# zakuro-ai/asr

Measured on AMD Instinct MI355X. Metric: utterances/sec (10 s, 161-bin) DS2 5x1024 BiGRU CTC train step, higher is better.
Workload: dtype bf16

## Files before the change

### asr_amd/_lib.py

```python
from __future__ import annotations

import ctypes as C
import os
from typing import Optional

_HERE = os.path.dirname(os.path.abspath(__file__))
LIB_PATH = os.environ.get("DS2_LIB_PATH") or os.path.join(_HERE, "lib", "libds2hip.so")

_lib: Optional[C.CDLL] = None

vp, i32, i64, f32, f64, sz = C.c_void_p, C.c_int, C.c_longlong, C.c_float, C.c_double, C.c_size_t

SIGNATURES = {
    "ds2_version": (C.c_char_p, []),
    "ds2_last_error": (C.c_char_p, []),
    "ds2_device_info": (i32, [C.POINTER(i32), C.POINTER(i32), C.c_char_p, i32]),
    "ds2_debug_flags": (i32, [vp, i32]),
    "ds2_rnn_ctx_init": (i32, [vp, vp, vp, vp]),
    "ds2_memset_async": (i32, [vp, i32, sz, vp]),
    "ds2_ablation_build": (i32, []),
    "ds2_rnn_persistent_status": (i32, [vp, vp]),
    "ds2_rnn_persistent_counters": (i32, [vp, vp]),
    "ds2_rnn_poison_if_starved": (i32, [vp, vp, sz, vp]),
    "ds2_rnn_poison_seen": (i32, [vp]),
# ... 32 lines not shown
    "ds2_bn1d_apply_f32": (i32, [vp, i32, vp, i32, i32, i32, vp, vp, vp, vp, f32, vp]),
    "ds2_bn1d_apply_bf16": (i32, [vp, i32, vp, i32, i32, i32, vp, vp, vp, vp, f32, vp]),
    "ds2_bn1d_bwd_f32": (i32, [vp, i32, vp, i32, vp, i32, i32, i32, vp, vp, vp, f32, vp, vp, vp, sz, vp]),
    "ds2_bn1d_bwd_xbf16": (i32, [vp, i32, vp, i32, vp, i32, i32, i32, vp, vp, vp, f32, vp, vp, vp, sz, vp]),
    "ds2_center_colstats": (i32, [vp, i32, vp, i32, vp, i32, vp, i32, i32, i32, vp, vp, vp, vp, vp, f32, vp, sz, vp]),
    "ds2_wih_fold_bf16": (i32, [vp, i32, vp, i32, i32, vp, vp, vp, vp, f32, vp, i32, vp, vp, vp, vp]),
    "ds2_scale_rank1_f32": (i32, [vp, i32, i32, i32, vp, vp, vp, vp]),
    "ds2_chanreduce_workspace_bytes": (sz, [i32]),
    "ds2_bn2d_stats_f32": (i32, [vp, i32, i32, i32, i32, vp, vp, vp, vp, f32, vp, sz, vp]),
    "ds2_bn2d_act_fwd_f32": (i32, [vp, vp, i32, i32, i32, i32, vp, vp, vp, vp, vp, f32, vp]),
    "ds2_bn2d_act_bwd_f32": (i32, [vp, vp, vp, i32, i32, i32, i32, vp, vp, vp, vp, vp, f32, vp, vp, vp, sz, vp]),
    "ds2_bn2d_act_fwd_fused": (i32, [vp, i32, i32, i32, vp, vp, vp, vp, vp, f32, vp, vp, vp, vp]),
    "ds2_bn2d_act_collapse": (i32, [vp, i32, i32, i32, vp, vp, vp, vp, vp, f32, vp, vp, i32, vp]),
    "ds2_bn2d_act_bwd_fused_workspace_bytes": (sz, [i32, i32, i32]),
    "ds2_bn2d_act_bwd_fused": (i32, [vp, vp, i32, i32, i32, vp, vp, vp, vp, vp, f32, vp, vp, vp, vp, vp, vp, vp, sz, vp]),
    "ds2_transpose_bft_f32": (i32, [vp, vp, i32, i32, i32, i32, vp]),
    "ds2_transpose2d_f32": (i32, [vp, i32, i64, vp, i32, i64, i32, i32, i32, vp]),
    "ds2_conv_dims": (None, [i32, i32, C.POINTER(i32), C.POINTER(i32), C.POINTER(i32)]),
    "ds2_conv_packed_floats": (sz, [i32]),
    "ds2_conv_pack_f32": (i32, [vp, vp, vp, vp, vp, vp]),
    "ds2_conv1_fwd_f32": (i32, [vp, vp, vp, vp, vp, i32, i32, i32, vp]),
    "ds2_conv2_fwd_f32": (i32, [vp, vp, vp, vp, vp, i32, i32, i32, vp]),
    "ds2_conv2_dgrad_f32": (i32, [vp, vp, vp, i32, i32, i32, vp]),
    "ds2_conv_wgrad_workspace_bytes": (sz, [i32, i32, i32]),
    "ds2_conv1_wgrad_f32": (i32, [vp, vp, vp, vp, i32, i32, i32, i32, vp, sz, vp]),
    "ds2_conv2_wgrad_f32": (i32, [vp, vp, vp, vp, i32, i32, i32, i32, vp, sz, vp]),
    "ds2_conv2_bf16_packed_bytes": (sz, [i32]),
    "ds2_conv2_pack_bf16": (i32, [vp, vp, vp, vp, vp]),
    "ds2_nhwc_bf16_f32": (i32, [vp, vp, i32, i32, i32, vp]),
    "ds2_conv2_fwd_bf16": (i32, [vp, vp, vp, vp, vp, i32, i32, i32, vp]),
# ... 58 lines not shown
    "ds2_ctc_hot_pack": (i32, [i32, i32, vp, vp, vp, vp, vp, vp, i32, vp, sz]),
    "ds2_ctc_hot_step": (i32, [vp, i32, i32, C.POINTER(i32), C.POINTER(f32)]),
    "ds2_ctc_beam_decode_hot_f32": (i32, [vp, i64, i64, i32, i32, i32, vp, i32, i32, i32, f32, vp, sz, i32, i32, i32, f32, f32, vp, vp, sz,
                                          vp, vp, vp, vp, vp, sz, vp]),
    "ds2_edit_distance_workspace_bytes": (sz, [i32, i64]),
    "ds2_edit_distance_i32": (i32, [vp, i64, vp, vp, vp, vp, i32, i64, vp, vp, sz, vp]),
    "ds2_edit_align_workspace_bytes": (sz, [i32, i64]),
    "ds2_edit_align_i32": (i32, [vp, i64, vp, vp, vp, vp, i32, i64, vp, vp, vp, vp, sz, vp]),
    "ds2_conv1_bf16_row_pitch": (i32, [i32]),
    "ds2_conv1_bf16_bytes": (sz, [i32, i32, i32, i32]),
    "ds2_conv1_pack_bf16": (i32, [vp, vp, vp]),
    "ds2_conv1_gather_bf16": (i32, [vp, vp, vp, i32, i32, i32, vp]),
    "ds2_conv1_fwd_bf16": (i32, [vp, vp, vp, vp, vp, i32, i32, i32, vp]),
    "ds2_conv1_wgrad_bf16_workspace_bytes": (sz, [i32, i32]),
    "ds2_conv1_wgrad_bf16": (i32, [vp, vp, vp, vp, i32, i32, i32, vp, sz, vp]),
    "ds2_spectrogram_frames": (i32, [i32, i32]),
    "ds2_spectrogram_workspace_bytes": (sz, [i32, i32, i32, i32]),
    "ds2_spectrogram_f32": (i32, [vp, i64, vp, i32, i32, i32, i32, vp, i32, i32, vp, vp, sz, vp]),
    "ds2_spectrogram_aug_workspace_bytes": (sz, [i32, i32, i32, i32]),
    "ds2_spectrogram_aug_f32": (i32, [vp, i64, vp, i32, i32, i32, i32, vp, i32, i32, vp, i64, vp, vp, vp, vp, vp, i32, vp, i32, vp, vp, sz,
                                      vp]),
    "ds2_tempo_sizes": (i32, [i32, f64, f64, f64, C.POINTER(i32), C.POINTER(i32), C.POINTER(i32)]),
    "ds2_tempo_out_samples": (i32, [i32, f64]),
    "ds2_tempo_workspace_bytes": (sz, [i32]),
    "ds2_tempo_gain_f32": (i32, [vp, i64, vp, vp, vp, i32, i32, f64, f64, f64, vp, i64, vp, vp, i32, vp, sz, vp]),
    "ds2_wave_unpack_f32": (i32, [vp, i64, i32, vp, vp, vp, i32, i32, vp, i64, vp]),
    "ds2_resample_out_samples": (i64, [i64, i32, i32]),
    "ds2_resample_tile_samples": (i32, []),
    "ds2_wave_resample_f32": (i32, [vp, i64, i32, vp, vp, vp, vp, vp, vp, vp, vp, i64, i32, i32, vp, i64, vp]),
    "ds2_reverb_max_taps": (i32, []),
# ... 57 lines not shown
```

### asr_amd/csrc/conv1_bf16.hip

```cpp
#include "common.h"
#include <type_traits>

namespace {

typedef __bf16 bf16x8 __attribute__((ext_vector_type(8)));
typedef unsigned int u32x4 __attribute__((ext_vector_type(4)));
typedef float f32x4_c1 __attribute__((ext_vector_type(4), aligned(4)));

constexpr int KD = 41, KTAPS = 11, PD = 20, PT = 5, CO = 32, NC = 16;

__device__ __attribute__((aligned(16))) float g_zero_c1[4] = {0.f, 0.f, 0.f, 0.f};

#ifdef DS2_C1_TRACE
__device__ unsigned long long g_c1_trace[8192 * 8];
#define C1T_DECL unsigned long long c1t_[8] = {0, 0, 0, 0, 0, 0, 0, 0}, c1t_last_ = __builtin_amdgcn_s_memtime()
#define C1T(k) do { const unsigned long long n_ = __builtin_amdgcn_s_memtime(); c1t_[k] += n_ - c1t_last_; c1t_last_ = n_; } while (0)
#define C1T_DUMP(blk) do { if (threadIdx.x == 0) for (int k_ = 0; k_ < 8; ++k_) g_c1_trace[(long long)(blk) * 8 + k_] = c1t_[k_]; } while (0)
#else
#define C1T_DECL
#define C1T(k)
#define C1T_DUMP(blk)
#endif

__global__ __launch_bounds__(256) void conv1_gather_kernel(const float* __restrict__ x, __bf16* __restrict__ X16, __bf16* __restrict__ X16T,
// ... 196 lines not shown

constexpr int W_TT = 64;
constexpr int W_PF = 4;
constexpr int W_PITCH = W_TT * 2 + 16;
constexpr int W_SLOT = NC * W_PITCH;
constexpr int W_NR = 44;
constexpr int W_DY = CO * W_PITCH;
constexpr int W_LDS = (W_NR + 1) * W_SLOT + 2 * W_DY;
constexpr int W_TILES = (KD + 1) / 2;
constexpr int W_TPW = (W_TILES + 3) / 4;

struct C1WArgs {
  const __bf16* X16T; const float* dy; const int* lens; float* part;
  int B, F, T, Tp, D1;
};

__global__ __launch_bounds__(256) void conv1_bf16_wgrad_kernel(C1WArgs a) {
  extern __shared__ __attribute__((aligned(16))) char lds[];
  char* ring = lds;
  char* zslot = lds + W_NR * W_SLOT;
  char* dyl = zslot + W_SLOT;
  const int tid = threadIdx.x, lane = tid & 63;
  const int wave = __builtin_amdgcn_readfirstlane(tid >> 6);
  const int l31 = lane & 31, half = lane >> 5;
  const int t0 = blockIdx.x * W_TT, b = blockIdx.y;
  const int len = a.lens ? min(a.lens[b], a.T) : a.T;
  float* out = a.part + ((long long)b * gridDim.x + blockIdx.x) * (CO * KD * KTAPS);

  f32x16 acc[W_TPW];
#pragma unroll
  for (int i = 0; i < W_TPW; ++i)
#pragma unroll
// ... 7 lines not shown
    auto dy_load = [&](int o, int k, f32x4& v) {
      const int co = k >> 4, tq = t0 + (k & 15) * 4;
      const bool row_ok = o < a.D1;
      const float* p = a.dy + (((long long)b * CO + co) * a.D1 + (row_ok ? o : 0)) * a.T + tq;
      const float* z = g_zero_c1;
      v.x = *((row_ok && tq < a.T) ? p : z);
      v.y = *((row_ok && tq + 1 < a.T) ? p + 1 : z);
      v.z = *((row_ok && tq + 2 < a.T) ? p + 2 : z);
      v.w = *((row_ok && tq + 3 < a.T) ? p + 3 : z);
    };
    auto dy_store = [&](int buf, int k, const f32x4& v) {
      typedef __bf16 bf16x4 __attribute__((ext_vector_type(4)));
      const int co = k >> 4, tq = (k & 15) * 4;
      *reinterpret_cast<bf16x4*>(dyl + buf * W_DY + co * W_PITCH + tq * 2) = bf16x4{(__bf16)v.x, (__bf16)v.y, (__bf16)v.z, (__bf16)v.w};
    };
    for (int c = tid; c < W_SLOT / 16; c += 256) *reinterpret_cast<u32x4*>(zslot + c * 16) = u32x4{0u, 0u, 0u, 0u};
    for (int c = tid; c < KD * 128; c += 256) {
      const int r = c >> 7, k = c & 127;
      *reinterpret_cast<u32x4*>(ring + r * W_SLOT + (k >> 3) * W_PITCH + (k & 7) * 16) = *reinterpret_cast<const u32x4*>(row_src(r - PD, k >> 3, k & 7));
    }
    {
      f32x4 v0, v1;
      dy_load(0, tid, v0);
      dy_load(0, tid + 256, v1);
      dy_store(0, tid, v0);
      dy_store(0, tid + 256, v1);
    }
    struct Regs { u32x4 nr; f32x4 d0, d1; };
    const int nrow = tid >> 7, nk = tid & 127;
    unsigned dyoff[2][4];
#pragma unroll
    for (int h = 0; h < 2; ++h) {
      const int k = tid + 256 * h, co = k >> 4, tq = t0 + (k & 15) * 4;
#pragma unroll
      for (int j = 0; j < 4; ++j) dyoff[h][j] = (unsigned)(((long long)co * a.D1 * a.T + min(tq + j, a.T - 1)) * 4);
    }
    const unsigned rowoff = (unsigned)((((long long)nrow * NC + (nk >> 3)) * a.Tp + t0 + (nk & 7) * 8) * 2);
    const char* dy_b = reinterpret_cast<const char*>(a.dy + (long long)b * CO * a.D1 * a.T);
    const char* x_b = reinterpret_cast<const char*>(a.X16T + (long long)b * a.F * NC * a.Tp);
    const int nrow_u = __builtin_amdgcn_readfirstlane(nrow);
    const bool full_tile = t0 + W_TT <= a.T;
    auto fetch = [&](int o, Regs& r, auto full_c) {
      const int f = 2 * o - 1 + PD + nrow_u;
      const bool ok = f < a.F;
      const char* xs = ok ? x_b + (long long)f * NC * a.Tp * 2 - (long long)nrow_u * NC * a.Tp * 2 : reinterpret_cast<const char*>(g_zero_c1);
      r.nr = *reinterpret_cast<const u32x4*>(xs + (ok ? rowoff : 0u));
      const char* ds_ = dy_b + (long long)min(o, a.D1 - 1) * a.T * 4;
      if constexpr (decltype(full_c)::value) {
        const f32x4_c1 q0 = *reinterpret_cast<const f32x4_c1*>(ds_ + dyoff[0][0]), q1 = *reinterpret_cast<const f32x4_c1*>(ds_ + dyoff[1][0]);
        r.d0 = f32x4{q0.x, q0.y, q0.z, q0.w};
        r.d1 = f32x4{q1.x, q1.y, q1.z, q1.w};
      } else {
        r.d0 = f32x4{*reinterpret_cast<const float*>(ds_ + dyoff[0][0]), *reinterpret_cast<const float*>(ds_ + dyoff[0][1]),
                     *reinterpret_cast<const float*>(ds_ + dyoff[0][2]), *reinterpret_cast<const float*>(ds_ + dyoff[0][3])};
        r.d1 = f32x4{*reinterpret_cast<const float*>(ds_ + dyoff[1][0]), *reinterpret_cast<const float*>(ds_ + dyoff[1][1]),
                     *reinterpret_cast<const float*>(ds_ + dyoff[1][2]), *reinterpret_cast<const float*>(ds_ + dyoff[1][3])};
      }
    };
    auto publish = [&](int o, const Regs& r) {
      if (o < a.D1) {
        const int slot = (2 * o - 1 + nrow + 2 * PD) % W_NR;
        *reinterpret_cast<u32x4*>(ring + slot * W_SLOT + (nk >> 3) * W_PITCH + (nk & 7) * 16) = r.nr;
        dy_store(o & 1, tid, r.d0);
        dy_store(o & 1, tid + 256, r.d1);
      }
    };
    auto compute = [&](int o) {
      const char* ap = dyl + (o & 1) * W_DY + l31 * W_PITCH + half * 16;
      const int cl = l31 & 15, kdl = l31 >> 4;
      const int s0 = (2 * o + 2 * wave + kdl) % W_NR;
      const char* bp[W_TPW];
#pragma unroll
      for (int i = 0; i < W_TPW; ++i) {
        const int kd = 2 * (wave + 4 * i) + kdl;
        int slot = s0 + 8 * i;
        slot -= (slot >= W_NR) ? W_NR : 0;
        slot -= (slot >= W_NR) ? W_NR : 0;
        bp[i] = (kd < KD ? ring + slot * W_SLOT : zslot) + cl * W_PITCH + half * 16;
      }
// ... 27 lines not shown
            fetch(o + k + W_PF, rs[k], full_c);
            C1T(1);
            compute(o + k);
            C1T(2);
            publish(o + k + 1, rs[(k + 1) % W_PF]);
            C1T(3);
            __syncthreads();
            C1T(4);
          }
        }
      }
      C1T_DUMP(4096 + (long long)blockIdx.y * gridDim.x + blockIdx.x);
    };
    if (full_tile) run(std::true_type{});
    else run(std::false_type{});
  }
#pragma unroll
  for (int i = 0; i < W_TPW; ++i) {
    const int j = wave + 4 * i;
    if (j < W_TILES) {
      const int kd = 2 * j + (l31 >> 4), c = l31 & 15;
      if (kd < KD && c < KTAPS) {
#pragma unroll
        for (int r = 0; r < 16; ++r) {
          const int co = (r & 3) + 8 * (r >> 2) + 4 * half;
          out[(co * KD + kd) * KTAPS + c] = acc[i][r];
        }
      }
    }
  }
// ... 92 lines not shown

extern "C" size_t ds2_conv1_wgrad_bf16_workspace_bytes(int B, int Tin) {
  const int T = (Tin + 2 * PT - KTAPS) / 2 + 1;
  return (size_t)B * ceil_div(T, W_TT) * CO * KD * KTAPS * sizeof(float);
}

extern "C" int ds2_conv1_wgrad_bf16(const void* X16T, const float* dy1, const int* lens_dev, float* dW1, int B, int F, int Tin, void* ws,
                                    size_t ws_bytes, void* stream) {
  DS2_REQUIRE(X16T && dy1 && dW1 && ws, "ds2_conv1_wgrad_bf16: null pointer");
  DS2_REQUIRE(ws_bytes >= ds2_conv1_wgrad_bf16_workspace_bytes(B, Tin), "ds2_conv1_wgrad_bf16: workspace too small");
  C1WArgs a{};
  a.X16T = (const __bf16*)X16T; a.dy = dy1; a.lens = lens_dev; a.part = (float*)ws;
  a.B = B; a.F = F; a.T = (Tin + 2 * PT - KTAPS) / 2 + 1; a.Tp = pad64(a.T); a.D1 = (F + 2 * PD - KD) / 2 + 1;
  static bool attr_set = false;
  if (!attr_set) {
    DS2_HIP(hipFuncSetAttribute((const void*)conv1_bf16_wgrad_kernel, hipFuncAttributeMaxDynamicSharedMemorySize, W_LDS));
    attr_set = true;
  }
  hipStream_t s = (hipStream_t)stream;
  const int ntt = ceil_div(a.T, W_TT);
  hipLaunchKernelGGL(conv1_bf16_wgrad_kernel, dim3(ntt, B), dim3(256), W_LDS, s, a);
  DS2_LAUNCH_CHECK("conv1_bf16_wgrad_kernel");
  hipLaunchKernelGGL(conv1_wgrad_reduce_kernel, dim3(ceil_div(CO * KD * KTAPS, 32)), dim3(256), 0, s, (const float*)ws, dW1, ntt * B);
  DS2_LAUNCH_CHECK("conv1_wgrad_reduce_kernel");
  return 0;
}
```

### asr_amd/csrc/norm.hip

```cpp
#include "common.h"
#include <algorithm>

namespace {

typedef float f32x4_dw __attribute__((ext_vector_type(4), aligned(4)));
typedef __bf16 nbf16x4 __attribute__((ext_vector_type(4)));
constexpr int BN_ROWS_PER_BLOCK = 32;
__device__ __forceinline__ f32x4 ld4(const float* __restrict__ p, int valid, bool vec) {
  f32x4 v = {0.f, 0.f, 0.f, 0.f};
  if (valid >= 4 && vec) {
    v = *reinterpret_cast<const f32x4*>(p);
  } else if (valid >= 4) {
    const f32x4_dw q = *reinterpret_cast<const f32x4_dw*>(p);
    v.x = q.x; v.y = q.y; v.z = q.z; v.w = q.w;
  } else {
    if (valid > 0) v.x = p[0];
    if (valid > 1) v.y = p[1];
    if (valid > 2) v.z = p[2];
    if (valid > 3) v.w = p[3];
  }
  return v;
}
__device__ __forceinline__ void st4(float* __restrict__ p, f32x4 v, int valid, bool vec) {
  if (valid >= 4 && vec) {
// ... 322 lines not shown
    } else {
#pragma unroll
      for (int j = 0; j < 4; ++j)
        if (tq0 + j < T) {
          y[j] = Yraw[row * T + tq0 + j];
          if (BWD) da[j] = dA[row * T + tq0 + j];
        }
    }
    float r[4];
#pragma unroll
    for (int j = 0; j < 4; ++j) {
      const bool live = tq0 + j < len;
      if (!BWD) {
        r[j] = live ? fminf(fmaxf((y[j] - mu) * (rs * ga) + be, 0.f), 20.f) : 0.f;
      } else {
        const float xh = (y[j] - mu) * rs;
        const float z = xh * ga + be;
        const float dz = (live && z > 0.f && z < 20.f) ? da[j] : 0.f;
        r[j] = live ? ga * rs * (dz - s0[c] * inv_count - xh * (s1[c] * inv_count)) : 0.f;
      }
      tile[c][tl4 + j] = r[j];
    }
    if (out_f32) {
      if (full4) *reinterpret_cast<f32x4u*>(out_f32 + row * T + tq0) = f32x4u{r[0], r[1], r[2], r[3]};
      else {
#pragma unroll
        for (int j = 0; j < 4; ++j) if (tq0 + j < T) out_f32[row * T + tq0 + j] = r[j];
      }
    }
    if (out_pad) {
#pragma unroll
      for (int j = 0; j < 4; ++j) if (tq0 + j < T) out_pad[row * Tp + 8 + tq0 + j] = (nbf16)r[j];
      if (blockIdx.x == 0 && l16 < 8) out_pad[row * Tp + l16] = (nbf16)0.f;
      if (blockIdx.x == gridDim.x - 1) for (int q = l16; T + 8 + q < Tp; q += 16) out_pad[row * Tp + T + 8 + q] = (nbf16)0.f;
// ... 651 lines not shown
                                      const float* var, const float* gamma, const float* beta, float eps, float* dgamma, float* dbeta,
                                      float* dbias, float* dy_f32, void* dy_pad, void* dy_nhwc, void* ws, size_t ws_bytes, void* stream) {
  DS2_REQUIRE(Y && dA && lens_dev && mean && var && gamma && beta && dgamma && dbeta && dbias, "ds2_bn2d_act_bwd_fused: null pointer");
  DS2_REQUIRE(ws && ws_bytes >= ds2_bn2d_act_bwd_fused_workspace_bytes(B, D, T), "ds2_bn2d_act_bwd_fused: workspace too small");
  const size_t red_bytes = ds2_chanreduce_workspace_bytes(32);
  int rc = chan_reduce_launch(1, Y, dA, B, 32, D, T, lens_dev, mean, var, gamma, beta, eps, 1, dbeta, dgamma, nullptr, nullptr, 0.f, ws,
                              red_bytes, (hipStream_t)stream);
  if (rc) return rc;
  float* part = reinterpret_cast<float*>(static_cast<char*>(ws) + red_bytes);
  const int Tp = (T + 16 + 7) / 8 * 8;
  const dim3 grid(ceil_div(T, 64), D, B);
  hipLaunchKernelGGL((bn2d_tile_kernel<true>), grid, dim3(256), 0, (hipStream_t)stream, Y, dA, B, D, T, Tp, lens_dev, mean, var, gamma, beta,
                     (const float*)dbeta, (const float*)dgamma, eps, 1.0f / ((float)B * D * T), dy_f32, (nbf16*)dy_pad, (nbf16*)dy_nhwc, part);
  DS2_LAUNCH_CHECK("bn2d_tile_kernel<bwd>");
  const long long nparts = (long long)grid.x * grid.y * grid.z;
  double* tmp = reinterpret_cast<double*>(reinterpret_cast<char*>(part) + align_up((size_t)nparts * 32 * sizeof(float), 16));
  const long long rpb = (nparts + CPF_BLOCKS - 1) / CPF_BLOCKS;
  const int nblk = (int)((nparts + rpb - 1) / rpb);
  hipLaunchKernelGGL(chan_part_finalize_kernel, dim3(nblk), dim3(256), 0, (hipStream_t)stream, (const float*)part, nparts, rpb, tmp, nblk, dbias, 0);
  hipLaunchKernelGGL(chan_part_finalize_kernel, dim3(1), dim3(256), 0, (hipStream_t)stream, (const float*)part, nparts, rpb, tmp, nblk, dbias, 1);
  DS2_LAUNCH_CHECK("chan_part_finalize_kernel");
  return 0;
}

extern "C" int ds2_transpose_bft_f32(const float* src, float* dst, int B, int F, int T, int dir, void* stream) {
  DS2_REQUIRE(src && dst && B > 0 && F > 0 && T > 0, "ds2_transpose_bft_f32: bad args");
  dim3 grid(ceil_div(T, 64), ceil_div(F, 64), B);
  hipLaunchKernelGGL(transpose_bft_kernel, grid, dim3(256), 0, (hipStream_t)stream, src, dst, B, F, T, dir);
  DS2_LAUNCH_CHECK("transpose_bft_kernel");
  return 0;
}

extern "C" int ds2_transpose2d_f32(const float* src, int ld_src, long long stride_src, float* dst, int ld_dst, long long stride_dst,
                                   int R, int Cc, int batch, void* stream) {
  DS2_REQUIRE(src && dst && R > 0 && Cc > 0 && batch > 0, "ds2_transpose2d_f32: bad args");
  dim3 grid(ceil_div(Cc, 32), ceil_div(R, 32), batch);
  hipLaunchKernelGGL(transpose2d_kernel, grid, dim3(256), 0, (hipStream_t)stream, src, ld_src, stride_src, dst, ld_dst, stride_dst, R, Cc);
// ... 4 lines not shown
```

### asr_amd/engine.py

```python
from __future__ import annotations

from dataclasses import dataclass, field
from typing import Dict, List, Optional

import torch

from . import _lib, ops

Tensor = torch.Tensor
import os as _os
def _tune(name: str, default: str) -> str:
    return _os.environ.get(name, default) if _os.environ.get("DS2_EXPERIMENTAL") == "1" else default


OVERLAP_MODE = _tune("DS2_OVERLAP", "2")
OVERLAP_WGRAD = OVERLAP_MODE == "1"
WGRAD_TN = _tune("DS2_WGRAD_TN", "1") != "0"
CONV_STATS = _tune("DS2_CONV_STATS", "1") != "0"
FUSE_BN_BWD = _tune("DS2_FUSE_BN_BWD", "1") != "0"
WGRAD_SIDE = _tune("DS2_WGRAD_SIDE", "sk")
WGRAD_IDLE = _tune("DS2_WGRAD_IDLE", "1") != "0"
WGRAD_IDLE_MIN_CUS = int(_tune("DS2_WGRAD_IDLE_MIN_CUS", "64"))
F32_GEMM = _os.environ.get("DS2_F32_GEMM", "split")


F32_RNN = _os.environ.get("DS2_F32_RNN", "split")


F32_CONV = _os.environ.get("DS2_F32_CONV", "split")
F32_CONV_FWD = _tune("DS2_F32_CONV_FWD", "f32")
CONV2_WGRAD = _tune("DS2_CONV2_WGRAD", "nhwc")
GX_BF16 = _tune("DS2_GX_BF16", "0") != "0"
WS_PREARM = _tune("DS2_WS_PREARM", "1") != "0"
BN_FOLD = _tune("DS2_BN_FOLD", "1") != "0"
BN_FOLD_IDLE = _tune("DS2_BN_FOLD_IDLE", "1") != "0"


def _f32_split_ok(M: int, N: int, K: int, H: int = 8) -> bool:
    return F32_GEMM == "split" and M >= 512 and N >= 256 and K >= 256 and K % 8 == 0 and N % 8 == 0 and H % 8 == 0


_BWD_PERSISTENT = {}
_SIDE = {}


def _idle_cus_beside_bwd_recurrence(device, B: int, H: int) -> int:
# ... 652 lines not shown
    cp = "conv.seq_module."
    da2 = ops.transpose_bft(dy, B, 32 * D2, T, to_tbf=False).view(B, 32, D2, T)
    m2, v2 = ctx.st2
    bf = cfg.precision == "bf16"
    if bf:
        _, dy2p, dy2n = ops.bn2d_act_bwd_fused(ctx.y2, da2, lens_dev, m2, v2, W[cp + "4.weight"], W[cp + "4.bias"], Gr[cp + "4.weight"],
                                               Gr[cp + "4.bias"], Gr[cp + "3.bias"], want_pad=CONV2_WGRAD != "nhwc", want_nhwc=True)
        del da2
        if CONV2_WGRAD == "nhwc":
            ops.conv2_wgrad_nhwc_bf16(ctx.a1p, dy2n, lens_dev, Gr[cp + "3.weight"])
        else:
            ops.conv2_wgrad_bf16(ctx.a1p, dy2p, lens_dev, Gr[cp + "3.weight"], T)
        da1 = ops.conv2_dgrad_bf16(dy2n, ctx.packs[1], ctx.packs[2], D1)
        del dy2p, dy2n
        m1, v1 = ctx.st1
        dy1, _, _ = ops.bn2d_act_bwd_fused(ctx.y1, da1, lens_dev, m1, v1, W[cp + "1.weight"], W[cp + "1.bias"], Gr[cp + "1.weight"],
                                           Gr[cp + "1.bias"], Gr[cp + "0.bias"], want_f32=True)
        del da1
        ops.conv1_wgrad_bf16(ctx.x16t, dy1, lens_dev, Gr[cp + "0.weight"], ctx.x.shape[3])
        ctx.x16t = None
    elif F32_CONV == "split":
        dy2, dy2p, dy2n = ops.bn2d_act_bwd_fused(ctx.y2, da2, lens_dev, m2, v2, W[cp + "4.weight"], W[cp + "4.bias"], Gr[cp + "4.weight"],
                                                 Gr[cp + "4.bias"], Gr[cp + "3.bias"], want_f32=True, want_pad=True, want_nhwc=True)
        del da2
        r2 = ops.bf16_residual(dy2)
        del dy2
        dy2p_lo, dy2n_lo = ops.padcast_bf16(r2), ops.nhwc_bf16(r2)
        r2 = ops.bf16_residual(ctx.a1)
        a1p = (ops.padcast_bf16(ctx.a1), ops.padcast_bf16(r2))
        del r2
        ph = ops.conv2_pack_bf16(W[cp + "3.weight"])
        pl = ops.conv2_pack_bf16(ops.bf16_residual(W[cp + "3.weight"]))
        g2 = Gr[cp + "3.weight"]
        gb, gc = torch.empty_like(g2), torch.empty_like(g2)
# ... 33 lines not shown
```

### asr_amd/ops.py

```python
from __future__ import annotations

import ctypes as C
import math
import threading
from typing import Optional, Tuple

import numpy as np
import torch

from . import _lib

Tensor = torch.Tensor
BN_EPS = 1e-5
BN_MOMENTUM = 0.1


def _ptr(t: Optional[Tensor]):
    return None if t is None else t.data_ptr()


def _stream():
    return torch.cuda.current_stream().cuda_stream


# ... 605 lines not shown
    _chk_f32(Y, dA, mean, var, gamma, beta, dgamma, dbeta, dbias)
    lib = _lib.load()
    B, Cc, D, T = Y.shape
    assert Cc == 32 and Y.is_contiguous() and dA.is_contiguous() and dA.shape == Y.shape
    d32 = torch.empty_like(Y) if want_f32 else None
    dpad = torch.empty(B, 32, D, lib.ds2_conv_padded_pitch(T), dtype=torch.bfloat16, device=Y.device) if want_pad else None
    dnh = torch.empty(B, D, T, 32, dtype=torch.bfloat16, device=Y.device) if want_nhwc else None
    wsb = lib.ds2_bn2d_act_bwd_fused_workspace_bytes(B, D, T)
    ws = _ws(wsb, Y.device)
    _lib.check(lib.ds2_bn2d_act_bwd_fused(Y.data_ptr(), dA.data_ptr(), B, D, T, lens_dev.data_ptr(), mean.data_ptr(), var.data_ptr(),
                                          gamma.data_ptr(), beta.data_ptr(), BN_EPS, dgamma.data_ptr(), dbeta.data_ptr(), dbias.data_ptr(),
                                          _ptr(d32), _ptr(dpad), _ptr(dnh), ws.data_ptr(), wsb, _stream()), "ds2_bn2d_act_bwd_fused")
    return d32, dpad, dnh


def chan_sum(Y: Tensor) -> Tensor:
    mean, _ = bn2d_stats(Y)
    B, Cc, D, T = Y.shape
    return mean * float(B * D * T)


def transpose_bft(src: Tensor, B: int, F: int, T: int, to_tbf: bool) -> Tensor:
    _chk_f32(src)
    dst = torch.empty((T, B, F) if to_tbf else (B, F, T), dtype=torch.float32, device=src.device)
    _lib.check(_lib.load().ds2_transpose_bft_f32(src.data_ptr(), dst.data_ptr(), B, F, T, 0 if to_tbf else 1, _stream()),
               "ds2_transpose_bft_f32")
    return dst


def transpose_batched(src: Tensor) -> Tensor:
# ... 99 lines not shown


def chanstats_from_partials(part: Tensor, count: int, run_mean: Optional[Tensor] = None, run_var: Optional[Tensor] = None):
    _chk_f32(part, run_mean, run_var)
    nblk, Cc, _ = part.shape
    mean = torch.empty(Cc, dtype=torch.float32, device=part.device)
    var = torch.empty_like(mean)
    lib = _lib.load()
    wsb = lib.ds2_chanstats_from_partials_workspace_bytes()
    ws = _ws(wsb, part.device)
    _lib.check(lib.ds2_chanstats_from_partials(part.data_ptr(), nblk, Cc, float(count), mean.data_ptr(), var.data_ptr(), _ptr(run_mean),
                                               _ptr(run_var), BN_MOMENTUM, ws.data_ptr(), wsb, _stream()), "ds2_chanstats_from_partials")
    return mean, var


def conv1_wgrad_bf16(X16T: Tensor, dy1: Tensor, lens_dev: Tensor, dW1: Tensor, Tin: int):
    _chk_f32(dy1, dW1)
    lib = _lib.load()
    B, F = X16T.shape[0], X16T.shape[1]
    wsb = lib.ds2_conv1_wgrad_bf16_workspace_bytes(B, Tin)
    ws = _ws(wsb, dy1.device)
    _lib.check(lib.ds2_conv1_wgrad_bf16(X16T.data_ptr(), dy1.data_ptr(), lens_dev.data_ptr(), dW1.data_ptr(), B, F, Tin, ws.data_ptr(), wsb,
                                        _stream()), "ds2_conv1_wgrad_bf16")


def conv2_pack_bf16(w2: Tensor):
    _chk_f32(w2)
    lib = _lib.load()
    bufs = [torch.empty(lib.ds2_conv2_bf16_packed_bytes(i), dtype=torch.uint8, device=w2.device) for i in range(3)]
    _lib.check(lib.ds2_conv2_pack_bf16(w2.data_ptr(), bufs[0].data_ptr(), bufs[1].data_ptr(), bufs[2].data_ptr(), _stream()),
               "ds2_conv2_pack_bf16")
    return tuple(bufs)


# ... 1040 lines not shown
```

### include/ds2hip.h

```cpp
#ifndef DS2HIP_H
#define DS2HIP_H

#include <stddef.h>
#include <stdint.h>

#ifdef __cplusplus
extern "C" {
#endif

const char* ds2_version(void);
const char* ds2_last_error(void);
int ds2_device_info(int* cu_count, int* wave_size, char* arch, int arch_len);
int ds2_ablation_build(void);

typedef struct ds2_rnn_ctx {
  int size;
  int persist_fwd, persist_bwd;
  int cooldown;
  int rearm_calls;
  int starved_total;
  int last_path;
  int last_bwd_kind;
  int debug_flags;
  int ws_prearmed;
// ... 66 lines not shown
                       float momentum, void* ws, size_t ws_bytes, void* stream);
int ds2_bn2d_act_fwd_f32(const float* Y, float* A, int B, int C, int D, int T, const int* lens_dev, const float* mean,
                         const float* var, const float* gamma, const float* beta, float eps, void* stream);
int ds2_bn2d_act_bwd_f32(const float* Y, const float* dA, float* dY, int B, int C, int D, int T, const int* lens_dev, const float* mean,
                         const float* var, const float* gamma, const float* beta, float eps, float* dgamma, float* dbeta, void* ws,
                         size_t ws_bytes, void* stream);

int ds2_bn2d_act_fwd_fused(const float* Y, int B, int D, int T, const int* lens_dev, const float* mean, const float* var,
                           const float* gamma, const float* beta, float eps, float* a_f32, void* a_pad, void* a_nhwc, void* stream);
int ds2_bn2d_act_collapse(const float* Y, int B, int D, int T, const int* lens_dev, const float* mean, const float* var,
                          const float* gamma, const float* beta, float eps, float* x_f32, void* x_bf16, int ld_bf, void* stream);
size_t ds2_bn2d_act_bwd_fused_workspace_bytes(int B, int D, int T);
int ds2_bn2d_act_bwd_fused(const float* Y, const float* dA, int B, int D, int T, const int* lens_dev, const float* mean,
                           const float* var, const float* gamma, const float* beta, float eps, float* dgamma, float* dbeta,
                           float* dbias, float* dy_f32, void* dy_pad, void* dy_nhwc, void* ws, size_t ws_bytes, void* stream);
int ds2_transpose_bft_f32(const float* src, float* dst, int B, int F, int T, int dir, void* stream);
int ds2_transpose2d_f32(const float* src, int ld_src, long long stride_src, float* dst, int ld_dst, long long stride_dst, int R, int Cc,
                        int batch, void* stream);

void ds2_conv_dims(int F, int Tin, int* D1, int* D2, int* T);
size_t ds2_conv_packed_floats(int which );
int ds2_conv_pack_f32(const float* w1, const float* w2, float* wpk1, float* wpk2, float* wpk2d, void* stream);
int ds2_conv1_fwd_f32(const float* x, const float* wpk1, const float* bias, const int* lens_dev, float* y1, int B, int F, int Tin,
                      void* stream);
int ds2_conv2_fwd_f32(const float* a1, const float* wpk2, const float* bias, const int* lens_dev, float* y2, int B, int D1, int T,
                      void* stream);
int ds2_conv2_dgrad_f32(const float* dy2, const float* wpk2d, float* da1, int B, int D1, int T, void* stream);
size_t ds2_conv_wgrad_workspace_bytes(int which , int B, int F);
int ds2_conv1_wgrad_f32(const float* x, const float* dy1, const int* lens_dev, float* dW1, int B, int F, int Tin, int accumulate, void* ws,
                        size_t ws_bytes, void* stream);
// ... 180 lines not shown
                               const int* seg_start_dev, const int* seg_len_dev, int S, int T_max, float* out, int* out_sizes,
                               void* stream);

int ds2_conv1_bf16_row_pitch(int T);
size_t ds2_conv1_bf16_bytes(int which, int B, int F, int T);
int ds2_conv1_pack_bf16(const float* w1, void* wp, void* stream);
int ds2_conv1_gather_bf16(const float* x, void* XB, void* X16T, int B, int F, int Tin, void* stream);
int ds2_conv1_fwd_bf16(const void* XB, const void* wp, const float* bias, const int* lens_dev, float* y1, int B, int F, int Tin,
                       void* stream);
int ds2_conv1_fwd_bf16_stat_blocks(int B, int F, int Tin);
int ds2_conv1_fwd_bf16_stats(const void* XB, const void* wp, const float* bias, const int* lens_dev, float* y1, int B, int F, int Tin,
                             float* stat_part, void* stream);
size_t ds2_conv1_wgrad_bf16_workspace_bytes(int B, int Tin);
int ds2_conv1_wgrad_bf16(const void* X16T, const float* dy1, const int* lens_dev, float* dW1, int B, int F, int Tin, void* ws,
                         size_t ws_bytes, void* stream);

int ds2_spectrogram_frames(int n_samples, int hop);
size_t ds2_spectrogram_workspace_bytes(int B, int T, int n_fft, int hop);
int ds2_spectrogram_f32(const float* audio, long long ld_audio, const int* n_samples_dev, int B, int T, int n_fft, int hop,
                        const float* basis, int pad_mode, int normalize, float* out, void* ws, size_t ws_bytes, void* stream);
size_t ds2_spectrogram_aug_workspace_bytes(int B, int T, int n_fft, int hop);
int ds2_spectrogram_aug_f32(const float* audio, long long ld_audio, const int* n_samples_dev, int B, int T, int n_fft, int hop,
                            const float* basis, int pad_mode, int normalize, const float* noise, long long noise_len,
                            const long long* noise_base, const int* noise_period, const int* noise_start, const float* noise_level,
                            const int* freq_masks, int n_freq_masks, const int* time_masks, int n_time_masks, float* out, void* ws,
                            size_t ws_bytes, void* stream);

int ds2_tempo_sizes(int sample_rate, double segment_ms, double search_ms, double overlap_ms, int* S, int* R, int* O);
int ds2_tempo_out_samples(int n, double f);
size_t ds2_tempo_workspace_bytes(int B);
// ... 33 lines not shown
```

Measured before the change: 2853.

## Fuse BN2d+activation backward into conv1 weight-gradient kernel

```diff
diff --git a/asr_amd/_lib.py b/asr_amd/_lib.py
--- a/asr_amd/_lib.py
+++ b/asr_amd/_lib.py
@@ -70,6 +70,7 @@
     "ds2_bn2d_act_collapse": (i32, [vp, i32, i32, i32, vp, vp, vp, vp, vp, f32, vp, vp, i32, vp]),
     "ds2_bn2d_act_bwd_fused_workspace_bytes": (sz, [i32, i32, i32]),
     "ds2_bn2d_act_bwd_fused": (i32, [vp, vp, i32, i32, i32, vp, vp, vp, vp, vp, f32, vp, vp, vp, vp, vp, vp, vp, sz, vp]),
+    "ds2_bn2d_act_bwd_sums": (i32, [vp, vp, i32, i32, i32, vp, vp, vp, vp, vp, f32, vp, vp, vp, sz, vp]),
     "ds2_transpose_bft_f32": (i32, [vp, vp, i32, i32, i32, i32, vp]),
     "ds2_transpose2d_f32": (i32, [vp, i32, i64, vp, i32, i64, i32, i32, i32, vp]),
     "ds2_conv_dims": (None, [i32, i32, C.POINTER(i32), C.POINTER(i32), C.POINTER(i32)]),
@@ -158,6 +159,8 @@
     "ds2_conv1_fwd_bf16": (i32, [vp, vp, vp, vp, vp, i32, i32, i32, vp]),
     "ds2_conv1_wgrad_bf16_workspace_bytes": (sz, [i32, i32]),
     "ds2_conv1_wgrad_bf16": (i32, [vp, vp, vp, vp, i32, i32, i32, vp, sz, vp]),
+    "ds2_conv1_wgrad_bn_bf16_workspace_bytes": (sz, [i32, i32, i32]),
+    "ds2_conv1_wgrad_bn_bf16": (i32, [vp, vp, vp, vp, vp, vp, vp, vp, vp, vp, f32, vp, vp, i32, i32, i32, vp, sz, vp]),
     "ds2_spectrogram_frames": (i32, [i32, i32]),
     "ds2_spectrogram_workspace_bytes": (sz, [i32, i32, i32, i32]),
     "ds2_spectrogram_f32": (i32, [vp, i64, vp, i32, i32, i32, i32, vp, i32, i32, vp, vp, sz, vp]),
diff --git a/asr_amd/csrc/bn2d_bwd.h b/asr_amd/csrc/bn2d_bwd.h
--- /dev/null
+++ b/asr_amd/csrc/bn2d_bwd.h
@@ -0,0 +1,13 @@
+#pragma once
+#include "common.h"
+
+__device__ __forceinline__ float bn2d_act_bwd_elem(float y, float da, bool live, float mu, float rs, float ga, float be, float gr, float s0,
+                                                   float m1, float inv_count) {
+  const float xh = (y - mu) * rs;
+  const float z = __builtin_fmaf(xh, ga, be);
+  const float dz = __int_as_float(__float_as_int(da) & -(int)(live && z > 0.f && z < 20.f));
+  return __int_as_float(__float_as_int(gr * __builtin_fmaf(-xh, m1, __builtin_fmaf(-s0, inv_count, dz))) & -(int)live);
+}
+
+size_t ds2i_chan_part_finalize_tmp_bytes(void);
+int ds2i_chan_part_finalize(const float* part, long long n, void* tmp, float* out, hipStream_t s);
diff --git a/asr_amd/csrc/conv1_bf16.hip b/asr_amd/csrc/conv1_bf16.hip
--- a/asr_amd/csrc/conv1_bf16.hip
+++ b/asr_amd/csrc/conv1_bf16.hip
@@ -1,4 +1,5 @@
 #include "common.h"
+#include "bn2d_bwd.h"
 #include <type_traits>
 
 namespace {
@@ -234,8 +235,25 @@
   const __bf16* X16T; const float* dy; const int* lens; float* part;
   int B, F, T, Tp, D1;
 };
-
-__global__ __launch_bounds__(256) void conv1_bf16_wgrad_kernel(C1WArgs a) {
+struct C1WBnArgs : C1WArgs {
+  const float* y; const float *mean, *var, *gamma, *beta, *s0, *s1;
+  float eps, inv_count;
+  float* chan_part;
+};
+
+__device__ __forceinline__ float row16_sum(float v) {
+  auto dpp = [](float x, auto ctrl) {
+    return __int_as_float(__builtin_amdgcn_update_dpp(0, __float_as_int(x), decltype(ctrl)::value, 0xf, 0xf, false));
+  };
+  v += dpp(v, std::integral_constant<int, 0xb1>{});
+  v += dpp(v, std::integral_constant<int, 0x4e>{});
+  v += dpp(v, std::integral_constant<int, 0x141>{});
+  v += dpp(v, std::integral_constant<int, 0x128>{});
+  return v;
+}
+
+template <bool FUSED>
+__global__ __launch_bounds__(256) void conv1_bf16_wgrad_kernel(std::conditional_t<FUSED, C1WBnArgs, C1WArgs> a) {
   extern __shared__ __attribute__((aligned(16))) char lds[];
   char* ring = lds;
   char* zslot = lds + W_NR * W_SLOT;
@@ -273,19 +291,47 @@
       const int co = k >> 4, tq = (k & 15) * 4;
       *reinterpret_cast<bf16x4*>(dyl + buf * W_DY + co * W_PITCH + tq * 2) = bf16x4{(__bf16)v.x, (__bf16)v.y, (__bf16)v.z, (__bf16)v.w};
     };
+    [[maybe_unused]] float cf[2][7];
+    [[maybe_unused]] const int l16 = tid & 15, nlive = len - (t0 + l16 * 4);
+    [[maybe_unused]] float* cpart = nullptr;
+    [[maybe_unused]] float inv_count = 0.f;
+    [[maybe_unused]] const unsigned cp_pitch = gridDim.x * CO * 4;
+    if constexpr (FUSED) {
+      inv_count = a.inv_count;
+#pragma unroll
+      for (int h = 0; h < 2; ++h) {
+        const int c = (tid >> 4) + 16 * h;
+        cf[h][0] = a.mean[c]; cf[h][1] = rsqrtf(a.var[c] + a.eps); cf[h][2] = a.gamma[c]; cf[h][3] = a.beta[c];
+        cf[h][4] = cf[h][2] * cf[h][1]; cf[h][5] = a.s0[c]; cf[h][6] = a.s1[c] * a.inv_count;
+      }
+      cpart = a.chan_part + (((long long)b * a.D1) * gridDim.x + blockIdx.x) * CO + (tid >> 4);
+    }
+    [[maybe_unused]] auto form = [&](int o, const f32x4& y0, const f32x4& g0, const f32x4& y1, const f32x4& g1) {
+      typedef __bf16 bf16x4 __attribute__((ext_vector_type(4)));
+#pragma unroll
+      for (int h = 0; h < 2; ++h) {
+        const f32x4 y = h ? y1 : y0, g = h ? g1 : g0;
+        float r[4];
+#pragma unroll
+        for (int j = 0; j < 4; ++j) r[j] = bn2d_act_bwd_elem(y[j], g[j], j < nlive, cf[h][0], cf[h][1], cf[h][2], cf[h][3], cf[h][4], cf[h][5], cf[h][6], inv_count);
+        *reinterpret_cast<bf16x4*>(dyl + (o & 1) * W_DY + ((tid >> 4) + 16 * h) * W_PITCH + l16 * 8) = bf16x4{(__bf16)r[0], (__bf16)r[1], (__bf16)r[2], (__bf16)r[3]};
+        const float sum = row16_sum(((r[0] + r[1]) + r[2]) + r[3]);
+        if (l16 == 0) *reinterpret_cast<float*>(reinterpret_cast<char*>(cpart + 16 * h) + (size_t)o * cp_pitch) = sum;
+      }
+    };
     for (int c = tid; c < W_SLOT / 16; c += 256) *reinterpret_cast<u32x4*>(zslot + c * 16) = u32x4{0u, 0u, 0u, 0u};
     for (int c = tid; c < KD * 128; c += 256) {
       const int r = c >> 7, k = c & 127;
       *reinterpret_cast<u32x4*>(ring + r * W_SLOT + (k >> 3) * W_PITCH + (k & 7) * 16) = *reinterpret_cast<const u32x4*>(row_src(r - PD, k >> 3, k & 7));
     }
-    {
+    if constexpr (!FUSED) {
       f32x4 v0, v1;
       dy_load(0, tid, v0);
       dy_load(0, tid + 256, v1);
       dy_store(0, tid, v0);
       dy_store(0, tid + 256, v1);
     }
-    struct Regs { u32x4 nr; f32x4 d0, d1; };
+    struct Regs { u32x4 nr; f32x4 d0, d1, y0, y1; };
     const int nrow = tid >> 7, nk = tid & 127;
     unsigned dyoff[2][4];
 #pragma unroll
@@ -297,6 +343,8 @@
     const unsigned rowoff = (unsigned)((((long long)nrow * NC + (nk >> 3)) * a.Tp + t0 + (nk & 7) * 8) * 2);
     const char* dy_b = reinterpret_cast<const char*>(a.dy + (long long)b * CO * a.D1 * a.T);
     const char* x_b = reinterpret_cast<const char*>(a.X16T + (long long)b * a.F * NC * a.Tp);
+    [[maybe_unused]] const char* y_b = nullptr;
+    if constexpr (FUSED) y_b = reinterpret_cast<const char*>(a.y + (long long)b * CO * a.D1 * a.T);
     const int nrow_u = __builtin_amdgcn_readfirstlane(nrow);
     const bool full_tile = t0 + W_TT <= a.T;
     auto fetch = [&](int o, Regs& r, auto full_c) {
@@ -315,13 +363,34 @@
         r.d1 = f32x4{*reinterpret_cast<const float*>(ds_ + dyoff[1][0]), *reinterpret_cast<const float*>(ds_ + dyoff[1][1]),
                      *reinterpret_cast<const float*>(ds_ + dyoff[1][2]), *reinterpret_cast<const float*>(ds_ + dyoff[1][3])};
       }
-    };
+      if constexpr (FUSED) {
+        const char* ys_ = y_b + (ds_ - dy_b);
+        if constexpr (decltype(full_c)::value) {
+          const f32x4_c1 q0 = *reinterpret_cast<const f32x4_c1*>(ys_ + dyoff[0][0]), q1 = *reinterpret_cast<const f32x4_c1*>(ys_ + dyoff[1][0]);
+          r.y0 = f32x4{q0.x, q0.y, q0.z, q0.w};
+          r.y1 = f32x4{q1.x, q1.y, q1.z, q1.w};
+        } else {
+          r.y0 = f32x4{*reinterpret_cast<const float*>(ys_ + dyoff[0][0]), *reinterpret_cast<const float*>(ys_ + dyoff[0][1]),
+                       *reinterpret_cast<const float*>(ys_ + dyoff[0][2]), *reinterpret_cast<const float*>(ys_ + dyoff[0][3])};
+          r.y1 = f32x4{*reinterpret_cast<const float*>(ys_ + dyoff[1][0]), *reinterpret_cast<const float*>(ys_ + dyoff[1][1]),
+                       *reinterpret_cast<const float*>(ys_ + dyoff[1][2]), *reinterpret_cast<const float*>(ys_ + dyoff[1][3])};
+        }
+      }
+    };
+    if constexpr (FUSED) {
+      Regs r0;
+      fetch(0, r0, std::false_type{});
+      form(0, r0.y0, r0.d0, r0.y1, r0.d1);
+    }
     auto publish = [&](int o, const Regs& r) {
       if (o < a.D1) {
         const int slot = (2 * o - 1 + nrow + 2 * PD) % W_NR;
         *reinterpret_cast<u32x4*>(ring + slot * W_SLOT + (nk >> 3) * W_PITCH + (nk & 7) * 16) = r.nr;
-        dy_store(o & 1, tid, r.d0);
-        dy_store(o & 1, tid + 256, r.d1);
+        if constexpr (FUSED) form(o, r.y0, r.d0, r.y1, r.d1);
+        else {
+          dy_store(o & 1, tid, r.d0);
+          dy_store(o & 1, tid + 256, r.d1);
+        }
       }
     };
     auto compute = [&](int o) {
@@ -379,6 +448,9 @@
     };
     if (full_tile) run(std::true_type{});
     else run(std::false_type{});
+  } else if constexpr (FUSED) {
+    for (int i = tid; i < a.D1 * CO; i += 256)
+      a.chan_part[(((long long)b * a.D1 + (i >> 5)) * gridDim.x + blockIdx.x) * CO + (i & 31)] = 0.f;
   }
 #pragma unroll
   for (int i = 0; i < W_TPW; ++i) {
@@ -501,14 +573,47 @@
   a.B = B; a.F = F; a.T = (Tin + 2 * PT - KTAPS) / 2 + 1; a.Tp = pad64(a.T); a.D1 = (F + 2 * PD - KD) / 2 + 1;
   static bool attr_set = false;
   if (!attr_set) {
-    DS2_HIP(hipFuncSetAttribute((const void*)conv1_bf16_wgrad_kernel, hipFuncAttributeMaxDynamicSharedMemorySize, W_LDS));
+    DS2_HIP(hipFuncSetAttribute((const void*)conv1_bf16_wgrad_kernel<false>, hipFuncAttributeMaxDynamicSharedMemorySize, W_LDS));
     attr_set = true;
   }
   hipStream_t s = (hipStream_t)stream;
   const int ntt = ceil_div(a.T, W_TT);
-  hipLaunchKernelGGL(conv1_bf16_wgrad_kernel, dim3(ntt, B), dim3(256), W_LDS, s, a);
+  hipLaunchKernelGGL(conv1_bf16_wgrad_kernel<false>, dim3(ntt, B), dim3(256), W_LDS, s, a);
   DS2_LAUNCH_CHECK("conv1_bf16_wgrad_kernel");
   hipLaunchKernelGGL(conv1_wgrad_reduce_kernel, dim3(ceil_div(CO * KD * KTAPS, 32)), dim3(256), 0, s, (const float*)ws, dW1, ntt * B);
   DS2_LAUNCH_CHECK("conv1_wgrad_reduce_kernel");
   return 0;
 }
+
+static size_t c1w_bn_part_bytes(int B, int F, int T) { return align_up((size_t)B * ((F + 2 * PD - KD) / 2 + 1) * ceil_div(T, W_TT) * CO * sizeof(float), 16); }
+extern "C" size_t ds2_conv1_wgrad_bn_bf16_workspace_bytes(int B, int F, int Tin) {
+  const int T = (Tin + 2 * PT - KTAPS) / 2 + 1;
+  return align_up(ds2_conv1_wgrad_bf16_workspace_bytes(B, Tin), 16) + c1w_bn_part_bytes(B, F, T) + ds2i_chan_part_finalize_tmp_bytes();
+}
+
+extern "C" int ds2_conv1_wgrad_bn_bf16(const void* X16T, const float* y1, const float* dA1, const int* lens_dev, const float* mean, const float* var,
+                                       const float* gamma, const float* beta, const float* s0, const float* s1, float eps, float* dW1, float* dbias,
+                                       int B, int F, int Tin, void* ws, size_t ws_bytes, void* stream) {
+  DS2_REQUIRE(X16T && y1 && dA1 && lens_dev && mean && var && gamma && beta && s0 && s1 && dW1 && dbias && ws, "ds2_conv1_wgrad_bn_bf16: null pointer");
+  DS2_REQUIRE(B > 0 && F > 0 && Tin > 0, "ds2_conv1_wgrad_bn_bf16: bad shape");
+  DS2_REQUIRE(ws_bytes >= ds2_conv1_wgrad_bn_bf16_workspace_bytes(B, F, Tin), "ds2_conv1_wgrad_bn_bf16: workspace too small");
+  C1WBnArgs a{};
+  a.X16T = (const __bf16*)X16T; a.dy = dA1; a.lens = lens_dev; a.part = (float*)ws;
+  a.B = B; a.F = F; a.T = (Tin + 2 * PT - KTAPS) / 2 + 1; a.Tp = pad64(a.T); a.D1 = (F + 2 * PD - KD) / 2 + 1;
+  a.y = y1; a.mean = mean; a.var = var; a.gamma = gamma; a.beta = beta; a.s0 = s0; a.s1 = s1;
+  a.eps = eps; a.inv_count = 1.0f / ((float)B * a.D1 * a.T);
+  char* cp = static_cast<char*>(ws) + align_up(ds2_conv1_wgrad_bf16_workspace_bytes(B, Tin), 16);
+  a.chan_part = reinterpret_cast<float*>(cp);
+  static bool attr_set = false;
+  if (!attr_set) {
+    DS2_HIP(hipFuncSetAttribute((const void*)conv1_bf16_wgrad_kernel<true>, hipFuncAttributeMaxDynamicSharedMemorySize, W_LDS));
+    attr_set = true;
+  }
+  hipStream_t s = (hipStream_t)stream;
+  const int ntt = ceil_div(a.T, W_TT);
+  hipLaunchKernelGGL(conv1_bf16_wgrad_kernel<true>, dim3(ntt, B), dim3(256), W_LDS, s, a);
+  DS2_LAUNCH_CHECK("conv1_bf16_wgrad_kernel<bn>");
+  hipLaunchKernelGGL(conv1_wgrad_reduce_kernel, dim3(ceil_div(CO * KD * KTAPS, 32)), dim3(256), 0, s, (const float*)ws, dW1, ntt * B);
+  DS2_LAUNCH_CHECK("conv1_wgrad_reduce_kernel");
+  return ds2i_chan_part_finalize(a.chan_part, (long long)B * a.D1 * ntt, cp + c1w_bn_part_bytes(B, F, a.T), dbias, s);
+}
diff --git a/asr_amd/csrc/norm.hip b/asr_amd/csrc/norm.hip
--- a/asr_amd/csrc/norm.hip
+++ b/asr_amd/csrc/norm.hip
@@ -1,4 +1,5 @@
 #include "common.h"
+#include "bn2d_bwd.h"
 #include <algorithm>
 
 namespace {
@@ -360,10 +361,7 @@
       if (!BWD) {
         r[j] = live ? fminf(fmaxf((y[j] - mu) * (rs * ga) + be, 0.f), 20.f) : 0.f;
       } else {
-        const float xh = (y[j] - mu) * rs;
-        const float z = xh * ga + be;
-        const float dz = (live && z > 0.f && z < 20.f) ? da[j] : 0.f;
-        r[j] = live ? ga * rs * (dz - s0[c] * inv_count - xh * (s1[c] * inv_count)) : 0.f;
+        r[j] = bn2d_act_bwd_elem(y[j], da[j], live, mu, rs, ga, be, ga * rs, s0[c], s1[c] * inv_count, inv_count);
       }
       tile[c][tl4 + j] = r[j];
     }
@@ -1045,13 +1043,28 @@
                      (const float*)dbeta, (const float*)dgamma, eps, 1.0f / ((float)B * D * T), dy_f32, (nbf16*)dy_pad, (nbf16*)dy_nhwc, part);
   DS2_LAUNCH_CHECK("bn2d_tile_kernel<bwd>");
   const long long nparts = (long long)grid.x * grid.y * grid.z;
-  double* tmp = reinterpret_cast<double*>(reinterpret_cast<char*>(part) + align_up((size_t)nparts * 32 * sizeof(float), 16));
+  return ds2i_chan_part_finalize(part, nparts, reinterpret_cast<char*>(part) + align_up((size_t)nparts * 32 * sizeof(float), 16), dbias,
+                                 (hipStream_t)stream);
+}
+
+size_t ds2i_chan_part_finalize_tmp_bytes(void) { return (size_t)CPF_BLOCKS * 32 * sizeof(double); }
+
+int ds2i_chan_part_finalize(const float* part, long long nparts, void* tmp_, float* out, hipStream_t s) {
+  double* tmp = static_cast<double*>(tmp_);
   const long long rpb = (nparts + CPF_BLOCKS - 1) / CPF_BLOCKS;
   const int nblk = (int)((nparts + rpb - 1) / rpb);
-  hipLaunchKernelGGL(chan_part_finalize_kernel, dim3(nblk), dim3(256), 0, (hipStream_t)stream, (const float*)part, nparts, rpb, tmp, nblk, dbias, 0);
-  hipLaunchKernelGGL(chan_part_finalize_kernel, dim3(1), dim3(256), 0, (hipStream_t)stream, (const float*)part, nparts, rpb, tmp, nblk, dbias, 1);
+  hipLaunchKernelGGL(chan_part_finalize_kernel, dim3(nblk), dim3(256), 0, s, part, nparts, rpb, tmp, nblk, out, 0);
+  hipLaunchKernelGGL(chan_part_finalize_kernel, dim3(1), dim3(256), 0, s, part, nparts, rpb, tmp, nblk, out, 1);
   DS2_LAUNCH_CHECK("chan_part_finalize_kernel");
   return 0;
+}
+
+extern "C" int ds2_bn2d_act_bwd_sums(const float* Y, const float* dA, int B, int D, int T, const int* lens_dev, const float* mean,
+                                     const float* var, const float* gamma, const float* beta, float eps, float* dgamma, float* dbeta,
+                                     void* ws, size_t ws_bytes, void* stream) {
+  DS2_REQUIRE(Y && dA && lens_dev && mean && var && gamma && beta && dgamma && dbeta, "ds2_bn2d_act_bwd_sums: null pointer");
+  return chan_reduce_launch(1, Y, dA, B, 32, D, T, lens_dev, mean, var, gamma, beta, eps, 1, dbeta, dgamma, nullptr, nullptr, 0.f, ws,
+                            ws_bytes, (hipStream_t)stream);
 }
 
 extern "C" int ds2_transpose_bft_f32(const float* src, float* dst, int B, int F, int T, int dir, void* stream) {
diff --git a/asr_amd/engine.py b/asr_amd/engine.py
--- a/asr_amd/engine.py
+++ b/asr_amd/engine.py
@@ -30,6 +30,7 @@
 F32_CONV = _os.environ.get("DS2_F32_CONV", "split")
 F32_CONV_FWD = _tune("DS2_F32_CONV_FWD", "f32")
 CONV2_WGRAD = _tune("DS2_CONV2_WGRAD", "nhwc")
+CONV1_WGRAD_BN = _tune("DS2_CONV1_WGRAD_BN", "1") != "0"
 GX_BF16 = _tune("DS2_GX_BF16", "0") != "0"
 WS_PREARM = _tune("DS2_WS_PREARM", "1") != "0"
 BN_FOLD = _tune("DS2_BN_FOLD", "1") != "0"
@@ -712,10 +713,16 @@
         da1 = ops.conv2_dgrad_bf16(dy2n, ctx.packs[1], ctx.packs[2], D1)
         del dy2p, dy2n
         m1, v1 = ctx.st1
-        dy1, _, _ = ops.bn2d_act_bwd_fused(ctx.y1, da1, lens_dev, m1, v1, W[cp + "1.weight"], W[cp + "1.bias"], Gr[cp + "1.weight"],
-                                           Gr[cp + "1.bias"], Gr[cp + "0.bias"], want_f32=True)
-        del da1
-        ops.conv1_wgrad_bf16(ctx.x16t, dy1, lens_dev, Gr[cp + "0.weight"], ctx.x.shape[3])
+        if CONV1_WGRAD_BN:
+            ops.bn2d_act_bwd_sums(ctx.y1, da1, lens_dev, m1, v1, W[cp + "1.weight"], W[cp + "1.bias"], Gr[cp + "1.weight"], Gr[cp + "1.bias"])
+            ops.conv1_wgrad_bf16(ctx.x16t, da1, lens_dev, Gr[cp + "0.weight"], ctx.x.shape[3],
+                                 bn=(ctx.y1, m1, v1, W[cp + "1.weight"], W[cp + "1.bias"], Gr[cp + "1.weight"], Gr[cp + "1.bias"], Gr[cp + "0.bias"]))
+            del da1
+        else:
+            dy1, _, _ = ops.bn2d_act_bwd_fused(ctx.y1, da1, lens_dev, m1, v1, W[cp + "1.weight"], W[cp + "1.bias"], Gr[cp + "1.weight"],
+                                               Gr[cp + "1.bias"], Gr[cp + "0.bias"], want_f32=True)
+            del da1
+            ops.conv1_wgrad_bf16(ctx.x16t, dy1, lens_dev, Gr[cp + "0.weight"], ctx.x.shape[3])
         ctx.x16t = None
     elif F32_CONV == "split":
         dy2, dy2p, dy2n = ops.bn2d_act_bwd_fused(ctx.y2, da2, lens_dev, m2, v2, W[cp + "4.weight"], W[cp + "4.bias"], Gr[cp + "4.weight"],
diff --git a/asr_amd/ops.py b/asr_amd/ops.py
--- a/asr_amd/ops.py
+++ b/asr_amd/ops.py
@@ -643,6 +643,18 @@
     return d32, dpad, dnh
 
 
+def bn2d_act_bwd_sums(Y: Tensor, dA: Tensor, lens_dev: Tensor, mean, var, gamma, beta, dgamma: Tensor, dbeta: Tensor):
+    _chk_f32(Y, dA, mean, var, gamma, beta, dgamma, dbeta)
+    lib = _lib.load()
+    B, Cc, D, T = Y.shape
+    assert Cc == 32 and Y.is_contiguous() and dA.is_contiguous() and dA.shape == Y.shape
+    wsb = lib.ds2_chanreduce_workspace_bytes(32)
+    ws = _ws(wsb, Y.device)
+    _lib.check(lib.ds2_bn2d_act_bwd_sums(Y.data_ptr(), dA.data_ptr(), B, D, T, lens_dev.data_ptr(), mean.data_ptr(), var.data_ptr(),
+                                         gamma.data_ptr(), beta.data_ptr(), BN_EPS, dgamma.data_ptr(), dbeta.data_ptr(), ws.data_ptr(), wsb,
+                                         _stream()), "ds2_bn2d_act_bwd_sums")
+
+
 def chan_sum(Y: Tensor) -> Tensor:
     mean, _ = bn2d_stats(Y)
     B, Cc, D, T = Y.shape
@@ -772,10 +784,21 @@
     return mean, var
 
 
-def conv1_wgrad_bf16(X16T: Tensor, dy1: Tensor, lens_dev: Tensor, dW1: Tensor, Tin: int):
+def conv1_wgrad_bf16(X16T: Tensor, dy1: Tensor, lens_dev: Tensor, dW1: Tensor, Tin: int, bn=None):
     _chk_f32(dy1, dW1)
     lib = _lib.load()
     B, F = X16T.shape[0], X16T.shape[1]
+    if bn is not None:
+        y1, mean, var, gamma, beta, dgamma, dbeta, dbias = bn
+        _chk_f32(y1, mean, var, gamma, beta, dgamma, dbeta, dbias)
+        D1, _, T = _lib.conv_dims(F, Tin)
+        assert y1.shape == (B, 32, D1, T) and dy1.shape == y1.shape and y1.is_contiguous() and dy1.is_contiguous()
+        wsb = lib.ds2_conv1_wgrad_bn_bf16_workspace_bytes(B, F, Tin)
+        ws = _ws(wsb, y1.device)
+        _lib.check(lib.ds2_conv1_wgrad_bn_bf16(X16T.data_ptr(), y1.data_ptr(), dy1.data_ptr(), lens_dev.data_ptr(), mean.data_ptr(), var.data_ptr(),
+                                               gamma.data_ptr(), beta.data_ptr(), dbeta.data_ptr(), dgamma.data_ptr(), BN_EPS, dW1.data_ptr(),
+                                               dbias.data_ptr(), B, F, Tin, ws.data_ptr(), wsb, _stream()), "ds2_conv1_wgrad_bn_bf16")
+        return
     wsb = lib.ds2_conv1_wgrad_bf16_workspace_bytes(B, Tin)
     ws = _ws(wsb, dy1.device)
     _lib.check(lib.ds2_conv1_wgrad_bf16(X16T.data_ptr(), dy1.data_ptr(), lens_dev.data_ptr(), dW1.data_ptr(), B, F, Tin, ws.data_ptr(), wsb,
diff --git a/include/ds2hip.h b/include/ds2hip.h
--- a/include/ds2hip.h
+++ b/include/ds2hip.h
@@ -104,6 +104,9 @@
 int ds2_bn2d_act_bwd_fused(const float* Y, const float* dA, int B, int D, int T, const int* lens_dev, const float* mean,
                            const float* var, const float* gamma, const float* beta, float eps, float* dgamma, float* dbeta,
                            float* dbias, float* dy_f32, void* dy_pad, void* dy_nhwc, void* ws, size_t ws_bytes, void* stream);
+int ds2_bn2d_act_bwd_sums(const float* Y, const float* dA, int B, int D, int T, const int* lens_dev, const float* mean, const float* var,
+                          const float* gamma, const float* beta, float eps, float* dgamma, float* dbeta, void* ws, size_t ws_bytes,
+                          void* stream);
 int ds2_transpose_bft_f32(const float* src, float* dst, int B, int F, int T, int dir, void* stream);
 int ds2_transpose2d_f32(const float* src, int ld_src, long long stride_src, float* dst, int ld_dst, long long stride_dst, int R, int Cc,
                         int batch, void* stream);
@@ -314,6 +317,10 @@
 size_t ds2_conv1_wgrad_bf16_workspace_bytes(int B, int Tin);
 int ds2_conv1_wgrad_bf16(const void* X16T, const float* dy1, const int* lens_dev, float* dW1, int B, int F, int Tin, void* ws,
                          size_t ws_bytes, void* stream);
+size_t ds2_conv1_wgrad_bn_bf16_workspace_bytes(int B, int F, int Tin);
+int ds2_conv1_wgrad_bn_bf16(const void* X16T, const float* y1, const float* dA1, const int* lens_dev, const float* mean, const float* var,
+                            const float* gamma, const float* beta, const float* s0, const float* s1, float eps, float* dW1, float* dbias,
+                            int B, int F, int Tin, void* ws, size_t ws_bytes, void* stream);
 
 int ds2_spectrogram_frames(int n_samples, int hop);
 size_t ds2_spectrogram_workspace_bytes(int B, int T, int n_fft, int hop);
```

Result: no change. 2870 (median of 6 runs) (+0.6%).
